# alibaba-mmai-research/CLIP-FSAR

Hardware: AMD Instinct MI355X
Metric: episodes/sec (5-way 1-shot, 8 frames, ViT-B/16) (higher is better)
Workload: dtype bf16; 1 GPU; BASELINE config[1]: 5-way 1-shot, 1 query/class, 8x224^2 frames, ViT-B/16, random-init CLIP weights, synthetic structured frames; frames_per_episode=80, precision=bf16, parallelism=episodes sharded over 1 rank(s); one all-gather of accuracies, launcher=single process

## Files before the change

clip-fsar_amd/csrc/gemm_vit.hip:

```cpp
#include <type_traits>
#include <utility>

#include "common.h"
#include "gemm_vit.h"

#include "gemm_vit_epi.h"

namespace {

template <typename TI, typename TO, int ACT, int MODE, int OPATH, int STORE, bool SHORTK = false, int MIW = 4>
__global__ __launch_bounds__(512, 2) void vit_gemm_kernel(VitGemmArgs p) {
    static_assert(!SHORTK || OPATH == 1, "K = 128 runs on the LDS-DMA path");
    static_assert(MIW == 4 || (MIW == 3 && !SHORTK), "tile height 256 or 192");
    constexpr int TMv = 64 * MIW;
    constexpr int WR = 32 * MIW;
    constexpr int NM = 2 * MIW;
    constexpr int NL = MIW + 2;
    constexpr bool WIDE = MODE == 6;
    constexpr bool HAS_RES = MODE == 1 || WIDE;
    constexpr bool LNFOLD = MODE == 2 || MODE == 4;
    constexpr bool HB = MODE == 4;
    extern __shared__ __attribute__((aligned(16))) char smem[];
    const int tid = threadIdx.x, lane = tid & 63;
    const int wave = __builtin_amdgcn_readfirstlane(tid >> 6);
    const int wm = wave >> 2, wn = wave & 3;
    const int lr = lane & 31, hi = lane >> 5;

// ... 219 lines not shown
    };
    u32x4 GX[4], GW[4];
    uint4 xfA[4], wfA[2], xfB[4], wfB[2];
    auto gloadX = [&](const unsigned (&ox)[4], int kt, auto J) __attribute__((always_inline)) {
        GX[decltype(J)::value] = *reinterpret_cast<const u32x4*>(p.A + (size_t)(kt >= p.nka ? kt - p.nka : kt) * akstride + ox[decltype(J)::value]);
    };
    auto gloadW = [&](const unsigned (&ow)[4], int kt, auto J) __attribute__((always_inline)) {
        GW[decltype(J)::value] = *reinterpret_cast<const u32x4*>(p.W + (size_t)kt * ROWB + ow[decltype(J)::value]);
    };
    auto swriteX = [&](int stage, auto J) __attribute__((always_inline)) {
        *reinterpret_cast<u32x4*>(smem + stage * STAGE + wr_off + decltype(J)::value * 8192) = GX[decltype(J)::value];
    };
    auto swriteW = [&](int stage, auto J) __attribute__((always_inline)) {
        *reinterpret_cast<u32x4*>(smem + stage * STAGE + TM * ROWB + wr_off + decltype(J)::value * 8192) = GW[decltype(J)::value];
    };
    auto dmaX = [&](const unsigned (&ox)[4], int kt, int stage, auto J) __attribute__((always_inline)) {
        const char* src = p.A + (size_t)(kt >= p.nka ? kt - p.nka : kt) * akstride + ox[decltype(J)::value];
        const unsigned dst = ldsw + (unsigned)stage * (unsigned)STAGE + (unsigned)decltype(J)::value * 8192u;
#ifdef CFSAR_DEV
        if (p.dbg & 4096) { glds16_asm_pol<1>(src, dst); return; }
        if (p.dbg & 16384) { glds16_asm_pol<2>(src, dst); return; }
#endif
        glds16_asm(src, dst);
    };
    auto dmaW = [&](const unsigned (&ow)[4], int kt, int stage, auto J) __attribute__((always_inline)) {
        const char* src = p.W + (size_t)kt * ROWB + ow[decltype(J)::value];
        const unsigned dst = ldsw + (unsigned)stage * (unsigned)STAGE + (unsigned)(TM * ROWB) + (unsigned)decltype(J)::value * 8192u;
#ifdef CFSAR_DEV
        if (p.dbg & 8192) { glds16_asm_pol<1>(src, dst); return; }
#endif
        glds16_asm(src, dst);
    };
    using T_ = std::true_type;
    using F_ = std::false_type;
    auto load_one = [&](int stage, int ss, auto J, uint4 (&xf)[4], uint4 (&wf)[2]) __attribute__((always_inline)) {
        constexpr int j = decltype(J)::value;
        const char* base = smem + stage * STAGE;
        const int x2 = ss << 5;
        constexpr int isx[6] = {1, 0, 1, 1, MIW == 4 ? 1 : 0, 0};
        constexpr int idx[6] = {0, 0, 1, 2, MIW == 4 ? 3 : 1, 1};
        if constexpr (isx[j] != 0) xf[idx[j]] = *reinterpret_cast<const uint4*>(base + (rdX[idx[j]] ^ x2));
        else wf[idx[j]] = *reinterpret_cast<const uint4*>(base + (rdW[idx[j]] ^ x2));
    };
    auto mfma_one = [&](auto J, uint4 (&xf)[4], uint4 (&wf)[2], auto ZERO) __attribute__((always_inline)) {
        constexpr int j = decltype(J)::value;
        constexpr int ni = j / MIW, mi = j % MIW;
        const f32x16 zero = {0.f, 0.f, 0.f, 0.f, 0.f, 0.f, 0.f, 0.f, 0.f, 0.f, 0.f, 0.f, 0.f, 0.f, 0.f, 0.f};
        const f32x16 c = decltype(ZERO)::value ? zero : acc[mi][ni];
        if constexpr (std::is_same<TI, _Float16>::value)
            acc[mi][ni] = __builtin_amdgcn_mfma_f32_32x32x16_f16(__builtin_bit_cast(f16x8, wf[ni]), __builtin_bit_cast(f16x8, xf[mi]), c, 0, 0, 0);
        else
            acc[mi][ni] = __builtin_amdgcn_mfma_f32_32x32x16_bf16(__builtin_bit_cast(bf16x8, wf[ni]), __builtin_bit_cast(bf16x8, xf[mi]), c, 0, 0, 0);
    };
    auto step = [&](int cur, int nxt, const unsigned (&ox)[4], const unsigned (&ow)[4], int ksrc, auto LOAD, auto WRITE, auto SYNC, auto FRAGS, auto ZERO, auto TAIL, int kstat = -1) __attribute__((always_inline)) {
        constexpr bool load = decltype(LOAD)::value, write = decltype(WRITE)::value, sync = decltype(SYNC)::value,
                       frags = decltype(FRAGS)::value, tail = decltype(TAIL)::value;
        static_for<NM>([&](auto J) {
            constexpr int j = decltype(J)::value;
            mfma_one(J, xfA, wfA, ZERO);
            if constexpr (j < NL) load_one(cur, 1, J, xfB, wfB);
            if constexpr (j >= NM - MIW) {
                if constexpr (OPATH == 0) { if constexpr (write) swriteX(nxt, std::integral_constant<int, j - (NM - MIW)>{}); }
                else if constexpr (OPATH == 1) { if constexpr (load) dmaX(ox, ksrc, nxt, std::integral_constant<int, j - (NM - MIW)>{}); }
            }
            __builtin_amdgcn_sched_barrier(0);
        });
        static_for<NM>([&](auto J) {
            constexpr int j = decltype(J)::value;
            mfma_one(J, xfB, wfB, F_{});
            if constexpr (j < NL) load_one(cur, 2, J, xfA, wfA);
            if constexpr (OPATH == 0) {
                if constexpr (j >= NM - MIW && load) gloadX(ox, ksrc, std::integral_constant<int, j - (NM - MIW)>{});
            } else if constexpr (OPATH == 1) {
                if constexpr (j >= NM - 4 && load) dmaW(ow, ksrc, nxt, std::integral_constant<int, j - (NM - 4)>{});
            }
            __builtin_amdgcn_sched_barrier(0);
        });
        static_for<NM>([&](auto J) {
            constexpr int j = decltype(J)::value;
            mfma_one(J, xfA, wfA, F_{});
            if constexpr (j < NL) load_one(cur, 3, J, xfB, wfB);
            if constexpr (j >= NM - 4 && OPATH == 0 && write) swriteW(nxt, std::integral_constant<int, j - (NM - 4)>{});
            __builtin_amdgcn_sched_barrier(0);
        });
        static_for<NM>([&](auto J) {
            constexpr int j = decltype(J)::value;
            mfma_one(J, xfB, wfB, F_{});
            if constexpr (j < 2) {
                if constexpr (OPATH == 0 && load) {
                    gloadW(ow, ksrc, std::integral_constant<int, 2 * j>{});
                    gloadW(ow, ksrc, std::integral_constant<int, 2 * j + 1>{});
                }
            } else if constexpr (frags) {
                load_one(nxt, 0, std::integral_constant<int, j - 2>{}, xfA, wfA);
                if constexpr (j == NM - 1 && NL > NM - 2) load_one(nxt, 0, std::integral_constant<int, NL - 1>{}, xfA, wfA);
            }
            if constexpr (tail && j == 2) tail_loads(m0, n0);
            if constexpr (kFuseStats && j == 2) stats_at(kstat);
            if constexpr (OPATH == 2 && load && j >= 2 && MIW == 4) {
                if constexpr (j < 6) dmaX(ox, ksrc, cur, std::integral_constant<int, j - 2>{});
                else {
                    dmaW(ow, ksrc, cur, std::integral_constant<int, 2 * (j - 6)>{});
                    dmaW(ow, ksrc, cur, std::integral_constant<int, 2 * (j - 6) + 1>{});
                }
            }
            if constexpr (OPATH == 2 && load && j >= 2 && MIW == 3) {
                if constexpr (j == 2) { dmaX(ox, ksrc, cur, std::integral_constant<int, 0>{}); dmaX(ox, ksrc, cur, std::integral_constant<int, 1>{}); }
                if constexpr (j == 3) { dmaX(ox, ksrc, cur, std::integral_constant<int, 2>{}); dmaW(ow, ksrc, cur, std::integral_constant<int, 0>{}); }
                if constexpr (j == 4) { dmaW(ow, ksrc, cur, std::integral_constant<int, 1>{}); dmaW(ow, ksrc, cur, std::integral_constant<int, 2>{}); }
                if constexpr (j == 5) { dmaW(ow, ksrc, cur, std::integral_constant<int, 3>{}); }
            }
            __builtin_amdgcn_sched_barrier(0);
            if constexpr (j == 1 && sync) {
                if constexpr (OPATH >= 1) asm volatile("s_waitcnt vmcnt(0)" ::: "memory");
#ifndef CFSAR_HIDDEN_TAIL_LOADS
                if constexpr (!frags && OPATH >= 1) tail_pin();
#endif
                __syncthreads();
                __builtin_amdgcn_sched_barrier(0);
            }
        });
    };
    origin(b, m0, n0);
    unsigned offX[4], offW[4];
    offsets(m0, n0, offX, offW);
    if constexpr (OPATH == 0) {
        static_for<MIW>([&](auto J) { gloadX(offX, 0, J); });
        static_for<4>([&](auto J) { gloadW(offW, 0, J); });
        static_for<MIW>([&](auto J) { swriteX(0, J); });
        static_for<4>([&](auto J) { swriteW(0, J); });
        static_for<MIW>([&](auto J) { gloadX(offX, 1, J); });
        static_for<4>([&](auto J) { gloadW(offW, 1, J); });
    } else {
        static_for<MIW>([&](auto J) { dmaX(offX, 0, 0, J); });
        static_for<4>([&](auto J) { dmaW(offW, 0, 0, J); });
        if constexpr (OPATH == 2) {
            static_for<MIW>([&](auto J) { dmaX(offX, 1, 1, J); });
            static_for<4>([&](auto J) { dmaW(offW, 1, 1, J); });
            asm volatile("s_waitcnt vmcnt(%0)" : : "n"(MIW + 4) : "memory");
        } else {
            asm volatile("s_waitcnt vmcnt(0)" ::: "memory");
        }
    }
    __syncthreads();
#ifdef CFSAR_DEV
    if (p.dbg & 32768) {
        if (wave >= 4) __builtin_amdgcn_s_setprio(1);
    }
    if (p.dbg & 65536) {
        if (wave < 4) __builtin_amdgcn_s_setprio(1);
    }
#endif
    int sb = 0;
// ... 2 lines not shown
    int trace_i = 0;
    if (p.dbg & 128) {
        const int n = ((blockIdx.x >> 3) & 31) * p.stagger_unit;
        for (int i = 0; i < n; ++i) __builtin_amdgcn_s_sleep(1);
        __syncthreads();
    }
#define CFSAR_TRACE(slot) do { if (p.trace && tid == 0 && trace_i < 64) p.trace[((size_t)blockIdx.x * 64 + trace_i) * 4 + (slot)] = (long long)__builtin_amdgcn_s_memrealtime(); } while (0)
#else
#define CFSAR_TRACE(slot) do { } while (0)
#endif
    for (;;) {
        const int bn = b + grid;
        const bool has_next = bn < nt;
        int m0n = m0, n0n = n0;
        if (has_next) origin(bn, m0n, n0n);
        static_for<NL>([&](auto J) { load_one(sb, 0, J, xfA, wfA); });
        CFSAR_TRACE(0);
        int kt = 0;
        u32x4 rv0[4] = {};
        auto residual_prefetch = [&]() __attribute__((always_inline)) {
            if constexpr (HAS_RES && !WIDE && OPATH >= 1) {
                const int mb_ = m0 + wm * WR, nb_ = n0 + wn * 64;
                const int ncl_ = nb_ + 64 <= p.N ? nb_ : p.N - 64;
                const int rr_ = lane >> 3, Q_ = lane & 7;
#pragma unroll
                for (int it = 0; it < 4; ++it) {
                    int row = mb_ + rr_ + it * 8;
                    row = row < p.M ? row : p.M - 1;
                    rv0[it] = *reinterpret_cast<const u32x4*>(reinterpret_cast<const char*>(p.res) + ((size_t)row * p.ldr + ncl_ + 8 * Q_) * 2);
                }
            }
        };
        if constexpr (OPATH == 0) {
            step(sb & 1, (sb + 1) & 1, offX, offW, 2, T_{}, T_{}, T_{}, T_{}, T_{}, F_{});
            for (kt = 1; kt < nk - 2; ++kt) step((sb + kt) & 1, (sb + kt + 1) & 1, offX, offW, kt + 2, T_{}, T_{}, T_{}, T_{}, F_{}, F_{});
            offsets(m0n, n0n, offX, offW);
            step((sb + kt) & 1, (sb + kt + 1) & 1, offX, offW, 0, T_{}, T_{}, T_{}, T_{}, F_{}, T_{});
            ++kt;
            step((sb + kt) & 1, (sb + kt + 1) & 1, offX, offW, 1, T_{}, T_{}, T_{}, F_{}, F_{}, F_{});
            asm volatile("s_waitcnt vmcnt(%0)" : : "n"(MIW + 4) : "memory");
        } else if constexpr (OPATH == 1 && SHORTK) {
            step(sb & 1, (sb + 1) & 1, offX, offW, 1, T_{}, F_{}, T_{}, T_{}, T_{}, T_{});
            kt = 1;
            offsets(m0n, n0n, offX, offW);
            residual_prefetch();
            step((sb + kt) & 1, (sb + kt + 1) & 1, offX, offW, 0, T_{}, F_{}, T_{}, F_{}, F_{}, F_{});
        } else if constexpr (OPATH == 1) {
            step(sb & 1, (sb + 1) & 1, offX, offW, 1, T_{}, F_{}, T_{}, T_{}, T_{}, F_{});
            for (kt = 1; kt < nk - 2; ++kt) step((sb + kt) & 1, (sb + kt + 1) & 1, offX, offW, kt + 1, T_{}, F_{}, T_{}, T_{}, F_{}, F_{});
            step((sb + kt) & 1, (sb + kt + 1) & 1, offX, offW, kt + 1, T_{}, F_{}, T_{}, T_{}, F_{}, T_{});
            ++kt;
            offsets(m0n, n0n, offX, offW);
            residual_prefetch();
            step((sb + kt) & 1, (sb + kt + 1) & 1, offX, offW, 0, T_{}, F_{}, T_{}, F_{}, F_{}, F_{});
        } else {
            step(sb & 1, (sb + 1) & 1, offX, offW, 2, T_{}, F_{}, T_{}, T_{}, T_{}, F_{}, 0);
            for (kt = 1; kt < nk - 2; ++kt) step((sb + kt) & 1, (sb + kt + 1) & 1, offX, offW, kt + 2, T_{}, F_{}, T_{}, T_{}, F_{}, F_{}, kt);
            offsets(m0n, n0n, offX, offW);
            step((sb + kt) & 1, (sb + kt + 1) & 1, offX, offW, 0, T_{}, F_{}, T_{}, T_{}, F_{}, T_{});
            ++kt;
            residual_prefetch();
// ... 42 lines not shown

int vit_pick_miw(int M, int tiles_n, int mode, int opath, int K, int dbg) {
    if (K == 128 || !vit_has_192(mode, opath)) return 4;
    const long long G = persistent_grid();
    const long long t256 = (long long)((M + 255) / 256) * tiles_n, t192 = (long long)((M + 191) / 192) * tiles_n;
    const long long r256 = ((t256 + G - 1) / G) * 256, r192 = ((t192 + G - 1) / G) * 192;
    int miw = r192 * 10 <= r256 * 9 ? 3 : 4;
#ifdef CFSAR_DEV
    if (dbg & (1 << 17)) miw = 3;
    if (dbg & (1 << 18)) miw = 4;
#endif
    (void)dbg;
    return miw;
}

template <typename TI, typename TO, int ACT, int MODE, int OPATH, int STORE, bool SHORTK, int MIW = 4>
int launch_inst2(const VitGemmArgs& a, hipStream_t s) {
    auto* fn = &vit_gemm_kernel<TI, TO, ACT, MODE, OPATH, STORE, SHORTK, MIW>;
    if (int rc = cfsar_ensure_lds(reinterpret_cast<const void*>(fn), LDS_BYTES, "cfsar_gemm(vit)")) return rc;
    const int grid = a.ntiles < persistent_grid() ? ((a.ntiles + 7) & ~7) : persistent_grid();
    hipLaunchKernelGGL(fn, dim3(grid), dim3(512), LDS_BYTES, s, a);
    return cfsar_check_launch("cfsar_gemm(vit)");
}

template <typename TI, typename TO, int ACT, int MODE, int OPATH, int STORE>
int launch_inst(const VitGemmArgs& a, hipStream_t s) {
    if (a.K == 128) return launch_inst2<TI, TO, ACT, MODE, 1, STORE, true>(a, s);
    if constexpr (vit_has_192(MODE, OPATH)) {
        if (a.miw == 3) return launch_inst2<TI, TO, ACT, MODE, OPATH, STORE, false, 3>(a, s);
    }
    return launch_inst2<TI, TO, ACT, MODE, OPATH, STORE, false>(a, s);
}

template <int OPATH, int STORE>
int launch_path(const VitGemmArgs& a, int mode, bool f16io, hipStream_t s) {
    if constexpr (STORE == 0) {
        if (mode == 5) return launch_inst<__bf16, __bf16, CFSAR_ACT_NONE, 1, OPATH, STORE>(a, s);
        if (mode == 6) return launch_inst<_Float16, _Float16, CFSAR_ACT_NONE, 6, OPATH, STORE>(a, s);
        if (mode == 1) {
            if (f16io) return launch_inst<_Float16, _Float16, CFSAR_ACT_NONE, 1, OPATH, STORE>(a, s);
            return launch_inst<__bf16, _Float16, CFSAR_ACT_NONE, 1, OPATH, STORE>(a, s);
        }
    } else {
        if (mode == 2) {
            if (f16io) {
                if (a.hb_tokens > 0) return -2;
                if (a.act == CFSAR_ACT_QUICKGELU) return launch_inst<_Float16, _Float16, CFSAR_ACT_QUICKGELU, 2, OPATH, STORE>(a, s);
                return launch_inst<_Float16, _Float16, CFSAR_ACT_NONE, 2, OPATH, STORE>(a, s);
            }
            if (a.act == CFSAR_ACT_QUICKGELU) return launch_inst<_Float16, __bf16, CFSAR_ACT_QUICKGELU, 2, OPATH, STORE>(a, s);
            if (a.hb_tokens > 0) return launch_inst<_Float16, __bf16, CFSAR_ACT_NONE, 4, OPATH, STORE>(a, s);
            return launch_inst<_Float16, __bf16, CFSAR_ACT_NONE, 2, OPATH, STORE>(a, s);
        }
        if (mode == 0) {
            if (a.act == CFSAR_ACT_QUICKGELU) return launch_inst<__bf16, __bf16, CFSAR_ACT_QUICKGELU, 0, OPATH, STORE>(a, s);
            if (a.relu) return launch_inst<__bf16, __bf16, kActRelu, 0, OPATH, STORE>(a, s);
            return launch_inst<__bf16, __bf16, CFSAR_ACT_NONE, 0, OPATH, STORE>(a, s);
        }
    }
    return cfsar_fail("cfsar_gemm (vit): internal: no instance of mode %d with store policy %d", mode, STORE);
}

}

#ifdef CFSAR_DEV
static int g_stagger_unit = 0;
static long long* g_trace = nullptr;
#endif
int cfsar_gemm_vit_try(const VitGemmCall& c, hipStream_t s) {
    const bool lnfold = c.rowstats != nullptr || c.part != nullptr;
    const bool f16io = lnfold ? c.out_dtype == CFSAR_F16 : c.in_dtype == CFSAR_F16;
    const bool f16res = !lnfold && c.out_dtype == CFSAR_F16 && c.res && c.res_dtype == CFSAR_F16 && c.act == CFSAR_ACT_NONE;
// ... 49 lines not shown
    a.ntiles = ((c.M + 64 * a.miw - 1) / (64 * a.miw)) * a.tiles_n;
    a.group = c.pol.group;
    a.colfast = c.pol.colfast;
    a.hb_tokens = c.hb_tokens; a.hb_heads = c.hb_heads; a.ha_tokens = c.ha_tokens;
    if (a.hb_tokens > 0 && !(lnfold && c.act == CFSAR_ACT_NONE && a.hb_tokens >= 128 && a.hb_heads > 0 && c.N == 3 * 64 * a.hb_heads &&
                             c.M % a.hb_tokens == 0))
        return cfsar_fail("cfsar_gemm_lnfold: head-blocked output needs act NONE, N = 192 heads, tokens >= 128, M a multiple of tokens");
    if (a.ha_tokens > 0 && !(f16res && a.ha_tokens >= 8 && c.M % a.ha_tokens == 0))
        return cfsar_fail("cfsar_gemm_residual_stats: head-blocked A needs M a multiple of tokens");
#ifdef CFSAR_DEV
    a.dbg = c.dbg;
    a.stagger_unit = g_stagger_unit;
    a.trace = g_trace;
#endif
    const int mode = lnfold ? 2 : (f16res ? (c.wide ? 6 : 1) : (bf16res ? 5 : 0));
    switch (c.pol.opath * 4 + c.pol.store) {
        case 0: return launch_path<0, 0>(a, mode, f16io, s);
        case 2: return launch_path<0, 2>(a, mode, f16io, s);
        case 8: return launch_path<2, 0>(a, mode, f16io, s);
        case 10: return launch_path<2, 2>(a, mode, f16io, s);
        default: return cfsar_fail("cfsar_gemm (vit): operand path %d / store policy %d is not built", c.pol.opath, c.pol.store);
    }
}

#ifdef CFSAR_DEV
static int g_force_opath = -1, g_force_dbg = 0;
#endif
VitPolicy cfsar_vit_policy(VitLaunchKind kind, int K) {
    const bool longk = K > 1024;
    const bool gemm = kind == kVitGemmPlain || kind == kVitGemmResidual;
    VitPolicy pol;
    pol.opath = longk ? 0 : 2;
    pol.store = (kind == kVitLnfold || kind == kVitGemmPlain) ? 2 : 0;
    pol.group = gemm ? 8 : (longk ? 16 : 6);
    pol.colfast = !gemm && longk;
// ... 12 lines not shown

namespace {
__global__ __launch_bounds__(256) void frame_means_from_colsums_kernel(const int* __restrict__ cs, __bf16* __restrict__ out, int wr,
                                                                       int tokens, int N) {
    const int f = blockIdx.y, n = blockIdx.x * 256 + threadIdx.x;
    if (n >= N) return;
    const int r0 = f * tokens, r1 = r0 + tokens - 1;
    long long s = 0;
    for (int b = r0 / wr; b <= r1 / wr; ++b) {
        const int j = f - (b * wr) / tokens;
        if (j == 0 || j == 1) s += cs[((size_t)b * 2 + j) * N + n];
    }
    out[(size_t)f * N + n] = (__bf16)((float)s * (1.0f / 4096.0f) / (float)tokens);
}
}

static int gemm_lnfold_impl(const void* x, const void* Wg, void* out, const float* cvec, const float* dvec,
                            const float* rowstats, int M, int N, int K, int lda, int ldw, int ldo, int act, int out_dtype, int hb_tokens,
                            int hb_heads, cfsar_stream_t stream, const float* partial = nullptr, int slots = 0, float eps = 0.f, int wsplit = 0,
                            const float* corr = nullptr, int corr_tokens = 0, void* colmean_out = nullptr, void* colsum_ws = nullptr) {
    CFSAR_REQUIRE(out_dtype == CFSAR_BF16 || out_dtype == CFSAR_F16, "cfsar_gemm_lnfold: out_dtype must be bf16 or fp16, got %d", out_dtype);
    CFSAR_REQUIRE(x && Wg && out && cvec && dvec && (rowstats || partial), "cfsar_gemm_lnfold: null pointer");
    CFSAR_REQUIRE(M > 0 && N > 0 && K >= 128 && K % 64 == 0 && N % 64 == 0, "cfsar_gemm_lnfold: bad shape M=%d N=%d K=%d (K %% 64, N %% 64, K >= 128)", M, N, K);
    CFSAR_REQUIRE(lda >= K && ldw >= (wsplit ? 2 * K : K) && ldo >= N && lda % 8 == 0 && ldw % 8 == 0 && ldo % 8 == 0, "cfsar_gemm_lnfold: bad leading dimension");
    CFSAR_REQUIRE(act == CFSAR_ACT_NONE || act == CFSAR_ACT_QUICKGELU, "cfsar_gemm_lnfold: bad act %d", act);
    const int ka_ = K;
    if (wsplit) K = 2 * K;
    VitGemmCall c;
    c.ka = ka_;
    c.corr_raw = corr_tokens < 0;
    if (corr_tokens < 0) corr_tokens = -corr_tokens;
    c.corr = corr; c.corr_tokens = corr_tokens;
    int miw_used = 4;
    c.colsum = colmean_out ? colsum_ws : nullptr; c.out_miw = &miw_used;
    c.A = x; c.W = Wg; c.out = out; c.bias = dvec; c.res = nullptr; c.rowstats = partial ? nullptr : rowstats; c.cvec = cvec; c.stats_out = nullptr;
    c.part = partial; c.part_slots = slots; c.part_eps = eps;
    c.M = M; c.N = N; c.K = K; c.lda = lda; c.ldw = ldw; c.ldo = ldo; c.ldr = 0;
    c.out_dtype = out_dtype; c.in_dtype = CFSAR_F16; c.res_dtype = CFSAR_F32; c.act = act; c.relu = 0;
    c.pol = cfsar_vit_policy(kVitLnfold, ka_); c.dbg = 0;
    c.hb_tokens = hb_tokens; c.hb_heads = hb_heads; c.ha_tokens = 0;
#ifdef CFSAR_DEV
    c.dbg = g_force_dbg;
#endif
    const int rc = cfsar_gemm_vit_try(c, static_cast<hipStream_t>(stream));
    if (rc == 0 && colmean_out) {
        const int frames = (M + corr_tokens - 1) / corr_tokens;
        hipLaunchKernelGGL(frame_means_from_colsums_kernel, dim3((unsigned)((N + 255) / 256), (unsigned)frames), dim3(256), 0,
                           static_cast<hipStream_t>(stream), static_cast<const int*>(colsum_ws), static_cast<__bf16*>(colmean_out),
                           32 * miw_used, corr_tokens, N);
        return cfsar_check_launch("cfsar_gemm_lnfold_hp(frame means)");
    }
    return rc == -2 ? cfsar_fail("cfsar_gemm_lnfold: operands too large for 32-bit offsets") : rc;
}

// ... 10 lines not shown
                  "cfsar_gemm_lnfold_heads: needs tokens >= 128, N = 192 heads, M a multiple of tokens (M=%d N=%d tokens=%d heads=%d)", M, N,
                  tokens, heads);
    return gemm_lnfold_impl(x, Wg, out, cvec, dvec, rowstats, M, N, K, lda, ldw, N, CFSAR_ACT_NONE, CFSAR_BF16, tokens, heads, stream);
}

static int lnfold_partials_impl(const void* x, const void* Wg, void* out, const float* cvec, const float* dvec,
                                const float* partial, int slots, float eps, float* rowstats_ws, int M, int N, int K, int lda,
                                int ldw, int ldo, int act, int out_dtype, int tokens, int heads, int wsplit, cfsar_stream_t stream,
                                const float* corr = nullptr, int corr_tokens = 0, void* colmean_out = nullptr, void* colsum_ws = nullptr) {
    CFSAR_REQUIRE(partial != nullptr && rowstats_ws != nullptr, "cfsar_gemm_lnfold_partials: null partials / workspace");
    CFSAR_REQUIRE(slots > 0 && slots * 64 == K, "cfsar_gemm_lnfold_partials: K=%d is not 64 x slots=%d", K, slots);
    int dbg = 0;
#ifdef CFSAR_DEV
    dbg = g_force_dbg;
#endif
    const int opath = cfsar_vit_policy(kVitLnfold, K).opath;
    const bool fused = !wsplit && opath == 2 && (slots == 12 || slots == 16) && vit_pick_miw(M, (N + TN - 1) / TN, 2, opath, K, dbg) == 3;
    if (!fused) {
        if (int rc = cfsar_ln_stats_finalize(partial, rowstats_ws, M, slots, K, eps, stream)) return rc;
        if (tokens > 0) return cfsar_gemm_lnfold_heads(x, Wg, out, cvec, dvec, rowstats_ws, M, N, K, lda, ldw, tokens, heads, stream);
        return gemm_lnfold_impl(x, Wg, out, cvec, dvec, rowstats_ws, M, N, K, lda, ldw, ldo, act, out_dtype, 0, 0, stream, nullptr, 0, 0.f, wsplit, corr, corr_tokens,
                                colmean_out, colsum_ws);
    }
    if (tokens > 0) {
        CFSAR_REQUIRE(tokens >= 128 && heads > 0 && N == 192 * heads && M % tokens == 0 && act == CFSAR_ACT_NONE && out_dtype == CFSAR_BF16,
                      "cfsar_gemm_lnfold_partials: head-blocked output needs tokens >= 128, N = 192 heads, M a multiple of tokens, act NONE, bf16");
        return gemm_lnfold_impl(x, Wg, out, cvec, dvec, nullptr, M, N, K, lda, ldw, N, act, out_dtype, tokens, heads, stream, partial, slots, eps);
    }
    return gemm_lnfold_impl(x, Wg, out, cvec, dvec, nullptr, M, N, K, lda, ldw, ldo, act, out_dtype, 0, 0, stream, partial, slots, eps, wsplit, corr, corr_tokens,
                            colmean_out, colsum_ws);
}
// ... 23 lines not shown

static int gemm_residual_stats_impl(const void* A, const void* W, void* x, const float* bias, float* stats_partial, int M,
                                    int N, int K, int lda, int ldw, int ldx, int in_dtype, int ha_tokens, cfsar_stream_t stream) {
    CFSAR_REQUIRE(in_dtype == CFSAR_BF16 || in_dtype == CFSAR_F16, "cfsar_gemm_residual_stats: in_dtype must be bf16 or fp16, got %d", in_dtype);
    CFSAR_REQUIRE(A && W && x && bias, "cfsar_gemm_residual_stats: null pointer");
    CFSAR_REQUIRE(M > 0 && N > 0 && K >= 128 && K % 64 == 0 && N % 64 == 0, "cfsar_gemm_residual_stats: bad shape M=%d N=%d K=%d", M, N, K);
    CFSAR_REQUIRE(lda >= K && ldw >= K && ldx >= N && lda % 8 == 0 && ldw % 8 == 0 && ldx % 8 == 0, "cfsar_gemm_residual_stats: bad leading dimension");
    VitGemmCall c;
    c.A = A; c.W = W; c.out = x; c.bias = bias; c.res = x; c.rowstats = nullptr; c.cvec = nullptr; c.stats_out = stats_partial;
    c.part = nullptr; c.part_slots = 0; c.part_eps = 0.f;
    c.M = M; c.N = N; c.K = K; c.lda = lda; c.ldw = ldw; c.ldo = ldx; c.ldr = ldx;
    c.out_dtype = CFSAR_F16; c.in_dtype = in_dtype; c.res_dtype = CFSAR_F16; c.act = CFSAR_ACT_NONE; c.relu = 0;
    c.pol = cfsar_vit_policy(kVitResidual, K); c.dbg = 0;
    c.hb_tokens = 0; c.hb_heads = 0; c.ha_tokens = ha_tokens;
#ifdef CFSAR_DEV
    c.dbg = g_force_dbg & ((1 << 17) | (1 << 18));
#endif
    const int rc = cfsar_gemm_vit_try(c, static_cast<hipStream_t>(stream));
    return rc == -2 ? cfsar_fail("cfsar_gemm_residual_stats: operands too large for 32-bit offsets") : rc;
}

extern "C" int cfsar_gemm_residual_stats(const void* A, const void* W, void* x, const float* bias, float* stats_partial, int M,
                                         int N, int K, int lda, int ldw, int ldx, int in_dtype, cfsar_stream_t stream) {
    return gemm_residual_stats_impl(A, W, x, bias, stats_partial, M, N, K, lda, ldw, ldx, in_dtype, 0, stream);
}

extern "C" int cfsar_gemm_residual_wide(const void* A, const void* W, void* x_hi, void* x_lo, const float* bias, float* stats_partial, int M,
                                        int N, int K, int wsplit, int lda, int ldw, int ldx, const float* corr, int corr_tokens,
                                        cfsar_stream_t stream) {
    CFSAR_REQUIRE(corr == nullptr || corr_tokens >= 128, "cfsar_gemm_residual_wide: the per-frame correction needs >= 128 tokens per frame");
    CFSAR_REQUIRE(A && W && x_hi && bias, "cfsar_gemm_residual_wide: null pointer");
    CFSAR_REQUIRE(M > 0 && N > 0 && K >= 128 && K % 64 == 0 && N % 64 == 0, "cfsar_gemm_residual_wide: bad shape M=%d N=%d K=%d", M, N, K);
    CFSAR_REQUIRE(wsplit >= 0 && wsplit <= 2, "cfsar_gemm_residual_wide: wsplit must be 0, 1 or 2, got %d", wsplit);
    CFSAR_REQUIRE(wsplit != 2 || corr == nullptr, "cfsar_gemm_residual_wide: wsplit = 2 carries the weights' second word itself (no per-frame correction)");
    const int Kt = wsplit == 2 ? 3 * K : (wsplit ? 2 * K : K);
    const int Ka = wsplit == 2 ? 2 * K : K;
    CFSAR_REQUIRE(lda >= Ka && ldw >= Kt && ldx >= N && lda % 8 == 0 && ldw % 8 == 0 && ldx % 8 == 0, "cfsar_gemm_residual_wide: bad leading dimension");
    VitGemmCall c;
    c.A = A; c.W = W; c.out = x_hi; c.bias = bias; c.res = x_hi; c.rowstats = nullptr; c.cvec = nullptr; c.stats_out = stats_partial;
    c.part = nullptr; c.part_slots = 0; c.part_eps = 0.f;
    c.M = M; c.N = N; c.K = Kt; c.lda = lda; c.ldw = ldw; c.ldo = ldx; c.ldr = ldx;
    c.out_dtype = CFSAR_F16; c.in_dtype = CFSAR_F16; c.res_dtype = CFSAR_F16; c.act = CFSAR_ACT_NONE; c.relu = 0;
    c.pol = cfsar_vit_policy(kVitWide, K); c.dbg = 0;
    c.hb_tokens = 0; c.hb_heads = 0; c.ha_tokens = 0;
    c.ka = Ka; c.wide = 1; c.res_lo = x_lo; c.corr = corr; c.corr_tokens = corr_tokens;
#ifdef CFSAR_DEV
    c.dbg = g_force_dbg & ((1 << 17) | (1 << 18));
#endif
    const int rc = cfsar_gemm_vit_try(c, static_cast<hipStream_t>(stream));
    return rc == -2 ? cfsar_fail("cfsar_gemm_residual_wide: operands too large for 32-bit offsets") : rc;
}

extern "C" int cfsar_gemm_residual_stats_heads(const void* A, const void* W, void* x, const float* bias, float* stats_partial, int M,
                                               int N, int K, int ldw, int ldx, int tokens, cfsar_stream_t stream) {
    CFSAR_REQUIRE(tokens >= 8 && M % tokens == 0, "cfsar_gemm_residual_stats_heads: M=%d is not a multiple of tokens=%d", M, tokens);
    return gemm_residual_stats_impl(A, W, x, bias, stats_partial, M, N, K, K, ldw, ldx, CFSAR_BF16, tokens, stream);
}
```

Before: 359.3 episodes/s.

## Add triple-buffered deep-operand ring to the early-DMA ViT GEMM pipeline

```diff
diff --git a/clip-fsar_amd/csrc/gemm_vit.hip b/clip-fsar_amd/csrc/gemm_vit.hip
--- a/clip-fsar_amd/csrc/gemm_vit.hip
+++ b/clip-fsar_amd/csrc/gemm_vit.hip
@@ -5,12 +5,15 @@
 #include "gemm_vit.h"
 
 #include "gemm_vit_epi.h"
+#include "gemm_vit_ring.h"
 
 namespace {
 
-template <typename TI, typename TO, int ACT, int MODE, int OPATH, int STORE, bool SHORTK = false, int MIW = 4>
+template <typename TI, typename TO, int ACT, int MODE, int OPATH, int STORE, bool SHORTK = false, int MIW = 4, int DEEP = 0>
 __global__ __launch_bounds__(512, 2) void vit_gemm_kernel(VitGemmArgs p) {
     static_assert(!SHORTK || OPATH == 1, "K = 128 runs on the LDS-DMA path");
+    static_assert(DEEP == 0 || (OPATH == 2 && MIW == 4 && !SHORTK), "the third operand buffer: early-DMA path, 256-row tiles");
+    static_assert(8 * EPI_SLAB == TM * ROWB, "the slab area holds one 256-row operand tile");
     static_assert(MIW == 4 || (MIW == 3 && !SHORTK), "tile height 256 or 192");
     constexpr int TMv = 64 * MIW;
     constexpr int WR = 32 * MIW;
@@ -260,18 +263,18 @@
     auto swriteW = [&](int stage, auto J) __attribute__((always_inline)) {
         *reinterpret_cast<u32x4*>(smem + stage * STAGE + TM * ROWB + wr_off + decltype(J)::value * 8192) = GW[decltype(J)::value];
     };
-    auto dmaX = [&](const unsigned (&ox)[4], int kt, int stage, auto J) __attribute__((always_inline)) {
+    auto dmaX = [&](const unsigned (&ox)[4], int kt, unsigned adst, auto J) __attribute__((always_inline)) {
         const char* src = p.A + (size_t)(kt >= p.nka ? kt - p.nka : kt) * akstride + ox[decltype(J)::value];
-        const unsigned dst = ldsw + (unsigned)stage * (unsigned)STAGE + (unsigned)decltype(J)::value * 8192u;
+        const unsigned dst = ldsw + adst + (unsigned)decltype(J)::value * 8192u;
 #ifdef CFSAR_DEV
         if (p.dbg & 4096) { glds16_asm_pol<1>(src, dst); return; }
         if (p.dbg & 16384) { glds16_asm_pol<2>(src, dst); return; }
 #endif
         glds16_asm(src, dst);
     };
-    auto dmaW = [&](const unsigned (&ow)[4], int kt, int stage, auto J) __attribute__((always_inline)) {
+    auto dmaW = [&](const unsigned (&ow)[4], int kt, unsigned wdst, auto J) __attribute__((always_inline)) {
         const char* src = p.W + (size_t)kt * ROWB + ow[decltype(J)::value];
-        const unsigned dst = ldsw + (unsigned)stage * (unsigned)STAGE + (unsigned)(TM * ROWB) + (unsigned)decltype(J)::value * 8192u;
+        const unsigned dst = ldsw + wdst + (unsigned)(TM * ROWB) + (unsigned)decltype(J)::value * 8192u;
 #ifdef CFSAR_DEV
         if (p.dbg & 8192) { glds16_asm_pol<1>(src, dst); return; }
 #endif
@@ -279,14 +282,15 @@
     };
     using T_ = std::true_type;
     using F_ = std::false_type;
-    auto load_one = [&](int stage, int ss, auto J, uint4 (&xf)[4], uint4 (&wf)[2]) __attribute__((always_inline)) {
+    auto load_one = [&](int aoff, int woff, int ss, auto J, uint4 (&xf)[4], uint4 (&wf)[2]) __attribute__((always_inline)) {
         constexpr int j = decltype(J)::value;
-        const char* base = smem + stage * STAGE;
+        const char* abase = smem + aoff;
+        const char* wbase = smem + woff;
         const int x2 = ss << 5;
         constexpr int isx[6] = {1, 0, 1, 1, MIW == 4 ? 1 : 0, 0};
         constexpr int idx[6] = {0, 0, 1, 2, MIW == 4 ? 3 : 1, 1};
-        if constexpr (isx[j] != 0) xf[idx[j]] = *reinterpret_cast<const uint4*>(base + (rdX[idx[j]] ^ x2));
-        else wf[idx[j]] = *reinterpret_cast<const uint4*>(base + (rdW[idx[j]] ^ x2));
+        if constexpr (isx[j] != 0) xf[idx[j]] = *reinterpret_cast<const uint4*>(abase + (rdX[idx[j]] ^ x2));
+        else wf[idx[j]] = *reinterpret_cast<const uint4*>(wbase + (rdW[idx[j]] ^ x2));
     };
     auto mfma_one = [&](auto J, uint4 (&xf)[4], uint4 (&wf)[2], auto ZERO) __attribute__((always_inline)) {
         constexpr int j = decltype(J)::value;
@@ -304,28 +308,28 @@
         static_for<NM>([&](auto J) {
             constexpr int j = decltype(J)::value;
             mfma_one(J, xfA, wfA, ZERO);
-            if constexpr (j < NL) load_one(cur, 1, J, xfB, wfB);
+            if constexpr (j < NL) load_one(cur * STAGE, cur * STAGE, 1, J, xfB, wfB);
             if constexpr (j >= NM - MIW) {
                 if constexpr (OPATH == 0) { if constexpr (write) swriteX(nxt, std::integral_constant<int, j - (NM - MIW)>{}); }
-                else if constexpr (OPATH == 1) { if constexpr (load) dmaX(ox, ksrc, nxt, std::integral_constant<int, j - (NM - MIW)>{}); }
+                else if constexpr (OPATH == 1) { if constexpr (load) dmaX(ox, ksrc, (unsigned)nxt * (unsigned)STAGE, std::integral_constant<int, j - (NM - MIW)>{}); }
             }
             __builtin_amdgcn_sched_barrier(0);
         });
         static_for<NM>([&](auto J) {
             constexpr int j = decltype(J)::value;
             mfma_one(J, xfB, wfB, F_{});
-            if constexpr (j < NL) load_one(cur, 2, J, xfA, wfA);
+            if constexpr (j < NL) load_one(cur * STAGE, cur * STAGE, 2, J, xfA, wfA);
             if constexpr (OPATH == 0) {
                 if constexpr (j >= NM - MIW && load) gloadX(ox, ksrc, std::integral_constant<int, j - (NM - MIW)>{});
             } else if constexpr (OPATH == 1) {
-                if constexpr (j >= NM - 4 && load) dmaW(ow, ksrc, nxt, std::integral_constant<int, j - (NM - 4)>{});
+                if constexpr (j >= NM - 4 && load) dmaW(ow, ksrc, (unsigned)nxt * (unsigned)STAGE, std::integral_constant<int, j - (NM - 4)>{});
             }
             __builtin_amdgcn_sched_barrier(0);
         });
         static_for<NM>([&](auto J) {
             constexpr int j = decltype(J)::value;
             mfma_one(J, xfA, wfA, F_{});
-            if constexpr (j < NL) load_one(cur, 3, J, xfB, wfB);
+            if constexpr (j < NL) load_one(cur * STAGE, cur * STAGE, 3, J, xfB, wfB);
             if constexpr (j >= NM - 4 && OPATH == 0 && write) swriteW(nxt, std::integral_constant<int, j - (NM - 4)>{});
             __builtin_amdgcn_sched_barrier(0);
         });
@@ -338,23 +342,23 @@
                     gloadW(ow, ksrc, std::integral_constant<int, 2 * j + 1>{});
                 }
             } else if constexpr (frags) {
-                load_one(nxt, 0, std::integral_constant<int, j - 2>{}, xfA, wfA);
-                if constexpr (j == NM - 1 && NL > NM - 2) load_one(nxt, 0, std::integral_constant<int, NL - 1>{}, xfA, wfA);
+                load_one(nxt * STAGE, nxt * STAGE, 0, std::integral_constant<int, j - 2>{}, xfA, wfA);
+                if constexpr (j == NM - 1 && NL > NM - 2) load_one(nxt * STAGE, nxt * STAGE, 0, std::integral_constant<int, NL - 1>{}, xfA, wfA);
             }
             if constexpr (tail && j == 2) tail_loads(m0, n0);
             if constexpr (kFuseStats && j == 2) stats_at(kstat);
             if constexpr (OPATH == 2 && load && j >= 2 && MIW == 4) {
-                if constexpr (j < 6) dmaX(ox, ksrc, cur, std::integral_constant<int, j - 2>{});
+                if constexpr (j < 6) dmaX(ox, ksrc, (unsigned)cur * (unsigned)STAGE, std::integral_constant<int, j - 2>{});
                 else {
-                    dmaW(ow, ksrc, cur, std::integral_constant<int, 2 * (j - 6)>{});
-                    dmaW(ow, ksrc, cur, std::integral_constant<int, 2 * (j - 6) + 1>{});
+                    dmaW(ow, ksrc, (unsigned)cur * (unsigned)STAGE, std::integral_constant<int, 2 * (j - 6)>{});
+                    dmaW(ow, ksrc, (unsigned)cur * (unsigned)STAGE, std::integral_constant<int, 2 * (j - 6) + 1>{});
                 }
             }
             if constexpr (OPATH == 2 && load && j >= 2 && MIW == 3) {
-                if constexpr (j == 2) { dmaX(ox, ksrc, cur, std::integral_constant<int, 0>{}); dmaX(ox, ksrc, cur, std::integral_constant<int, 1>{}); }
-                if constexpr (j == 3) { dmaX(ox, ksrc, cur, std::integral_constant<int, 2>{}); dmaW(ow, ksrc, cur, std::integral_constant<int, 0>{}); }
-                if constexpr (j == 4) { dmaW(ow, ksrc, cur, std::integral_constant<int, 1>{}); dmaW(ow, ksrc, cur, std::integral_constant<int, 2>{}); }
-                if constexpr (j == 5) { dmaW(ow, ksrc, cur, std::integral_constant<int, 3>{}); }
+                if constexpr (j == 2) { dmaX(ox, ksrc, (unsigned)cur * (unsigned)STAGE, std::integral_constant<int, 0>{}); dmaX(ox, ksrc, (unsigned)cur * (unsigned)STAGE, std::integral_constant<int, 1>{}); }
+                if constexpr (j == 3) { dmaX(ox, ksrc, (unsigned)cur * (unsigned)STAGE, std::integral_constant<int, 2>{}); dmaW(ow, ksrc, (unsigned)cur * (unsigned)STAGE, std::integral_constant<int, 0>{}); }
+                if constexpr (j == 4) { dmaW(ow, ksrc, (unsigned)cur * (unsigned)STAGE, std::integral_constant<int, 1>{}); dmaW(ow, ksrc, (unsigned)cur * (unsigned)STAGE, std::integral_constant<int, 2>{}); }
+                if constexpr (j == 5) { dmaW(ow, ksrc, (unsigned)cur * (unsigned)STAGE, std::integral_constant<int, 3>{}); }
             }
             __builtin_amdgcn_sched_barrier(0);
             if constexpr (j == 1 && sync) {
@@ -363,6 +367,79 @@
                 if constexpr (!frags && OPATH >= 1) tail_pin();
 #endif
                 __syncthreads();
+                __builtin_amdgcn_sched_barrier(0);
+            }
+        });
+    };
+
+    auto d_off = [&](int buf) __attribute__((always_inline)) -> int {
+        int off = buf == vit_ring::kSlab ? (DEEP == 2 ? EPI_OFF - TM * ROWB : EPI_OFF) : buf * STAGE;
+        asm volatile("" : "+s"(off));
+        return off;
+    };
+    auto step_deep = [&](int k, int sb_, const unsigned (&ox)[4], const unsigned (&ow)[4], auto KIND, auto KREP) __attribute__((always_inline)) {
+        constexpr int kind = decltype(KIND)::value;
+        using ZERO = std::integral_constant<bool, kind == 0>;
+        constexpr vit_ring::Step rd = vit_ring::step(decltype(KREP)::value, vit_ring::kRepTiles);
+        static_assert(kind == (rd.d_tile[1] != vit_ring::kNone ? 0 : rd.leave_d_tiles ? (rd.d_tile[0] != vit_ring::kNone ? 1 : 2) : (rd.d_dst[0] == 0 ? 3 : 4)), "step kind and ring step disagree");
+        const vit_ring::Step r = vit_ring::step(k, nk);
+        const int dcur = d_off(rd.d_read), scur = ((r.s_read + sb_) & 1) * STAGE;
+        const int dnxt = d_off(rd.d_next), snxt = ((r.s_next + sb_) & 1) * STAGE;
+        const int acur = DEEP == 1 ? dcur : scur, wcur = DEEP == 1 ? scur : dcur;
+        const int anxt = DEEP == 1 ? dnxt : snxt, wnxt = DEEP == 1 ? snxt : dnxt;
+        const int st = r.s_tile >= nk ? r.s_tile - nk : r.s_tile;
+        const unsigned sdst = (unsigned)(((r.s_dst + sb_) & 1) * STAGE);
+        auto issueS = [&](auto J) __attribute__((always_inline)) {
+            if constexpr (DEEP == 1) dmaW(ow, st, sdst, J); else dmaX(ox, st, sdst, J);
+        };
+        auto issueD = [&](int which, auto J) __attribute__((always_inline)) {
+            const int dt = r.d_tile[which] >= nk ? r.d_tile[which] - nk : r.d_tile[which];
+            const unsigned ddst = (unsigned)d_off(rd.d_dst[which]);
+            if constexpr (DEEP == 1) dmaX(ox, dt, ddst, J); else dmaW(ow, dt, ddst, J);
+        };
+        static_for<NM>([&](auto J) {
+            mfma_one(J, xfA, wfA, ZERO{});
+            if constexpr (decltype(J)::value < NL) load_one(acur, wcur, 1, J, xfB, wfB);
+            __builtin_amdgcn_sched_barrier(0);
+        });
+        static_for<NM>([&](auto J) {
+            mfma_one(J, xfB, wfB, F_{});
+            if constexpr (decltype(J)::value < NL) load_one(acur, wcur, 2, J, xfA, wfA);
+            __builtin_amdgcn_sched_barrier(0);
+        });
+        static_for<NM>([&](auto J) {
+            mfma_one(J, xfA, wfA, F_{});
+            if constexpr (decltype(J)::value < NL) load_one(acur, wcur, 3, J, xfB, wfB);
+            __builtin_amdgcn_sched_barrier(0);
+        });
+        static_for<NM>([&](auto J) {
+            constexpr int j = decltype(J)::value;
+            mfma_one(J, xfB, wfB, F_{});
+            if constexpr (j >= 2 && kind != 4) load_one(anxt, wnxt, 0, std::integral_constant<int, j - 2>{}, xfA, wfA);
+            if constexpr (kind == 3 && j == 2) tail_loads(m0, n0);
+            if constexpr (kind == 0 && j >= 2) {
+                constexpr int q = 2 * ((j - 2) & 1);
+                if constexpr (j < 4) { issueS(std::integral_constant<int, q>{}); issueS(std::integral_constant<int, q + 1>{}); }
+                else { issueD((j - 4) >> 1, std::integral_constant<int, q>{}); issueD((j - 4) >> 1, std::integral_constant<int, q + 1>{}); }
+            }
+            if constexpr (kind != 0 && j >= 2) {
+                if constexpr (j < 6) issueS(std::integral_constant<int, j - 2>{});
+                else if constexpr (kind != 2) { issueD(0, std::integral_constant<int, 2 * (j - 6)>{}); issueD(0, std::integral_constant<int, 2 * (j - 6) + 1>{}); }
+            }
+            __builtin_amdgcn_sched_barrier(0);
+            if constexpr (j == 1) {
+                if constexpr (kind == 1 || kind == 2) {
+                    asm volatile("s_waitcnt vmcnt(%0)" : : "n"(MIW) : "memory");
+                    asm volatile("s_waitcnt lgkmcnt(0)" ::: "memory");
+                    __builtin_amdgcn_s_barrier();
+                    asm volatile("" ::: "memory");
+                } else {
+                    asm volatile("s_waitcnt vmcnt(0)" ::: "memory");
+#ifndef CFSAR_HIDDEN_TAIL_LOADS
+                    if constexpr (kind == 4) tail_pin();
+#endif
+                    __syncthreads();
+                }
                 __builtin_amdgcn_sched_barrier(0);
             }
         });
@@ -378,11 +455,11 @@
         static_for<MIW>([&](auto J) { gloadX(offX, 1, J); });
         static_for<4>([&](auto J) { gloadW(offW, 1, J); });
     } else {
-        static_for<MIW>([&](auto J) { dmaX(offX, 0, 0, J); });
-        static_for<4>([&](auto J) { dmaW(offW, 0, 0, J); });
+        static_for<MIW>([&](auto J) { dmaX(offX, 0, 0u, J); });
+        static_for<4>([&](auto J) { dmaW(offW, 0, 0u, J); });
         if constexpr (OPATH == 2) {
-            static_for<MIW>([&](auto J) { dmaX(offX, 1, 1, J); });
-            static_for<4>([&](auto J) { dmaW(offW, 1, 1, J); });
+            static_for<MIW>([&](auto J) { dmaX(offX, 1, (unsigned)STAGE, J); });
+            static_for<4>([&](auto J) { dmaW(offW, 1, (unsigned)STAGE, J); });
             asm volatile("s_waitcnt vmcnt(%0)" : : "n"(MIW + 4) : "memory");
         } else {
             asm volatile("s_waitcnt vmcnt(0)" ::: "memory");
@@ -415,7 +492,9 @@
         const bool has_next = bn < nt;
         int m0n = m0, n0n = n0;
         if (has_next) origin(bn, m0n, n0n);
-        static_for<NL>([&](auto J) { load_one(sb, 0, J, xfA, wfA); });
+        static_for<NL>([&](auto J) {
+            load_one(DEEP == 1 ? 0 : sb * STAGE, DEEP == 2 ? 0 : sb * STAGE, 0, J, xfA, wfA);
+        });
         CFSAR_TRACE(0);
         int kt = 0;
         u32x4 rv0[4] = {};
@@ -446,6 +525,25 @@
             offsets(m0n, n0n, offX, offW);
             residual_prefetch();
             step((sb + kt) & 1, (sb + kt + 1) & 1, offX, offW, 0, T_{}, F_{}, T_{}, F_{}, F_{}, F_{});
+        } else if constexpr (DEEP != 0) {
+            using I0 = std::integral_constant<int, 0>; using I1 = std::integral_constant<int, 1>; using I2 = std::integral_constant<int, 2>;
+            using I3 = std::integral_constant<int, 3>; using I4 = std::integral_constant<int, 4>; using I5 = std::integral_constant<int, 5>;
+            constexpr int RT = vit_ring::kRepTiles;
+            step_deep(0, sb, offX, offW, I0{}, I0{});
+            step_deep(1, sb, offX, offW, I1{}, I4{});
+            step_deep(2, sb, offX, offW, I1{}, I5{});
+            for (kt = 3; kt < nk - 3; kt += 3) {
+                step_deep(kt, sb, offX, offW, I1{}, I3{});
+                step_deep(kt + 1, sb, offX, offW, I1{}, I4{});
+                step_deep(kt + 2, sb, offX, offW, I1{}, I5{});
+            }
+            step_deep(kt, sb, offX, offW, I2{}, std::integral_constant<int, RT - 3>{});
+            ++kt;
+            offsets(m0n, n0n, offX, offW);
+            step_deep(kt, sb, offX, offW, I3{}, std::integral_constant<int, RT - 2>{});
+            ++kt;
+            residual_prefetch();
+            step_deep(kt, sb, offX, offW, I4{}, std::integral_constant<int, RT - 1>{});
         } else if constexpr (OPATH == 1) {
             step(sb & 1, (sb + 1) & 1, offX, offW, 1, T_{}, F_{}, T_{}, T_{}, T_{}, F_{});
             for (kt = 1; kt < nk - 2; ++kt) step((sb + kt) & 1, (sb + kt + 1) & 1, offX, offW, kt + 1, T_{}, F_{}, T_{}, T_{}, F_{}, F_{});
@@ -518,9 +616,19 @@
     return miw;
 }
 
-template <typename TI, typename TO, int ACT, int MODE, int OPATH, int STORE, bool SHORTK, int MIW = 4>
+int vit_pick_deep(int opath, int miw, int K, bool fused_stats, int dbg) {
+    int deep = (opath == 2 && miw == 4 && K != 128 && !fused_stats && vit_ring::eligible(K / 64)) ? 1 : 0;
+#ifdef CFSAR_DEV
+    if (deep && (dbg & (1 << 23))) deep = 0;
+    if (deep && (dbg & (1 << 24))) deep = 2;
+#endif
+    (void)dbg;
+    return deep;
+}
+
+template <typename TI, typename TO, int ACT, int MODE, int OPATH, int STORE, bool SHORTK, int MIW = 4, int DEEP = 0>
 int launch_inst2(const VitGemmArgs& a, hipStream_t s) {
-    auto* fn = &vit_gemm_kernel<TI, TO, ACT, MODE, OPATH, STORE, SHORTK, MIW>;
+    auto* fn = &vit_gemm_kernel<TI, TO, ACT, MODE, OPATH, STORE, SHORTK, MIW, DEEP>;
     if (int rc = cfsar_ensure_lds(reinterpret_cast<const void*>(fn), LDS_BYTES, "cfsar_gemm(vit)")) return rc;
     const int grid = a.ntiles < persistent_grid() ? ((a.ntiles + 7) & ~7) : persistent_grid();
     hipLaunchKernelGGL(fn, dim3(grid), dim3(512), LDS_BYTES, s, a);
@@ -528,38 +636,49 @@
 }
 
 template <typename TI, typename TO, int ACT, int MODE, int OPATH, int STORE>
-int launch_inst(const VitGemmArgs& a, hipStream_t s) {
+int launch_inst(const VitGemmArgs& a, int deep, hipStream_t s) {
     if (a.K == 128) return launch_inst2<TI, TO, ACT, MODE, 1, STORE, true>(a, s);
     if constexpr (vit_has_192(MODE, OPATH)) {
         if (a.miw == 3) return launch_inst2<TI, TO, ACT, MODE, OPATH, STORE, false, 3>(a, s);
     }
+#ifdef CFSAR_DEV
+    constexpr bool kRing = OPATH == 2;
+#else
+    constexpr bool kRing = OPATH == 2 && !(MODE == 0 && ACT == CFSAR_ACT_QUICKGELU);
+#endif
+    if constexpr (kRing) {
+        if (deep == 1) return launch_inst2<TI, TO, ACT, MODE, OPATH, STORE, false, 4, 1>(a, s);
+#ifdef CFSAR_DEV
+        if (deep == 2) return launch_inst2<TI, TO, ACT, MODE, OPATH, STORE, false, 4, 2>(a, s);
+#endif
+    }
     return launch_inst2<TI, TO, ACT, MODE, OPATH, STORE, false>(a, s);
 }
 
 template <int OPATH, int STORE>
-int launch_path(const VitGemmArgs& a, int mode, bool f16io, hipStream_t s) {
+int launch_path(const VitGemmArgs& a, int deep, int mode, bool f16io, hipStream_t s) {
     if constexpr (STORE == 0) {
-        if (mode == 5) return launch_inst<__bf16, __bf16, CFSAR_ACT_NONE, 1, OPATH, STORE>(a, s);
-        if (mode == 6) return launch_inst<_Float16, _Float16, CFSAR_ACT_NONE, 6, OPATH, STORE>(a, s);
+        if (mode == 5) return launch_inst<__bf16, __bf16, CFSAR_ACT_NONE, 1, OPATH, STORE>(a, deep, s);
+        if (mode == 6) return launch_inst<_Float16, _Float16, CFSAR_ACT_NONE, 6, OPATH, STORE>(a, deep, s);
         if (mode == 1) {
-            if (f16io) return launch_inst<_Float16, _Float16, CFSAR_ACT_NONE, 1, OPATH, STORE>(a, s);
-            return launch_inst<__bf16, _Float16, CFSAR_ACT_NONE, 1, OPATH, STORE>(a, s);
+            if (f16io) return launch_inst<_Float16, _Float16, CFSAR_ACT_NONE, 1, OPATH, STORE>(a, deep, s);
+            return launch_inst<__bf16, _Float16, CFSAR_ACT_NONE, 1, OPATH, STORE>(a, deep, s);
         }
     } else {
         if (mode == 2) {
             if (f16io) {
                 if (a.hb_tokens > 0) return -2;
-                if (a.act == CFSAR_ACT_QUICKGELU) return launch_inst<_Float16, _Float16, CFSAR_ACT_QUICKGELU, 2, OPATH, STORE>(a, s);
-                return launch_inst<_Float16, _Float16, CFSAR_ACT_NONE, 2, OPATH, STORE>(a, s);
-            }
-            if (a.act == CFSAR_ACT_QUICKGELU) return launch_inst<_Float16, __bf16, CFSAR_ACT_QUICKGELU, 2, OPATH, STORE>(a, s);
-            if (a.hb_tokens > 0) return launch_inst<_Float16, __bf16, CFSAR_ACT_NONE, 4, OPATH, STORE>(a, s);
-            return launch_inst<_Float16, __bf16, CFSAR_ACT_NONE, 2, OPATH, STORE>(a, s);
+                if (a.act == CFSAR_ACT_QUICKGELU) return launch_inst<_Float16, _Float16, CFSAR_ACT_QUICKGELU, 2, OPATH, STORE>(a, deep, s);
+                return launch_inst<_Float16, _Float16, CFSAR_ACT_NONE, 2, OPATH, STORE>(a, deep, s);
+            }
+            if (a.act == CFSAR_ACT_QUICKGELU) return launch_inst<_Float16, __bf16, CFSAR_ACT_QUICKGELU, 2, OPATH, STORE>(a, deep, s);
+            if (a.hb_tokens > 0) return launch_inst<_Float16, __bf16, CFSAR_ACT_NONE, 4, OPATH, STORE>(a, deep, s);
+            return launch_inst<_Float16, __bf16, CFSAR_ACT_NONE, 2, OPATH, STORE>(a, deep, s);
         }
         if (mode == 0) {
-            if (a.act == CFSAR_ACT_QUICKGELU) return launch_inst<__bf16, __bf16, CFSAR_ACT_QUICKGELU, 0, OPATH, STORE>(a, s);
-            if (a.relu) return launch_inst<__bf16, __bf16, kActRelu, 0, OPATH, STORE>(a, s);
-            return launch_inst<__bf16, __bf16, CFSAR_ACT_NONE, 0, OPATH, STORE>(a, s);
+            if (a.act == CFSAR_ACT_QUICKGELU) return launch_inst<__bf16, __bf16, CFSAR_ACT_QUICKGELU, 0, OPATH, STORE>(a, deep, s);
+            if (a.relu) return launch_inst<__bf16, __bf16, kActRelu, 0, OPATH, STORE>(a, deep, s);
+            return launch_inst<__bf16, __bf16, CFSAR_ACT_NONE, 0, OPATH, STORE>(a, deep, s);
         }
     }
     return cfsar_fail("cfsar_gemm (vit): internal: no instance of mode %d with store policy %d", mode, STORE);
@@ -639,11 +758,12 @@
     a.trace = g_trace;
 #endif
     const int mode = lnfold ? 2 : (f16res ? (c.wide ? 6 : 1) : (bf16res ? 5 : 0));
+    const int deep = vit_pick_deep(c.pol.opath, a.miw, c.K, c.part != nullptr, c.dbg);
     switch (c.pol.opath * 4 + c.pol.store) {
-        case 0: return launch_path<0, 0>(a, mode, f16io, s);
-        case 2: return launch_path<0, 2>(a, mode, f16io, s);
-        case 8: return launch_path<2, 0>(a, mode, f16io, s);
-        case 10: return launch_path<2, 2>(a, mode, f16io, s);
+        case 0: return launch_path<0, 0>(a, deep, mode, f16io, s);
+        case 2: return launch_path<0, 2>(a, deep, mode, f16io, s);
+        case 8: return launch_path<2, 0>(a, deep, mode, f16io, s);
+        case 10: return launch_path<2, 2>(a, deep, mode, f16io, s);
         default: return cfsar_fail("cfsar_gemm (vit): operand path %d / store policy %d is not built", c.pol.opath, c.pol.store);
     }
 }
@@ -686,6 +806,8 @@
     out[(size_t)f * N + n] = (__bf16)((float)s * (1.0f / 4096.0f) / (float)tokens);
 }
 }
+
+static VitPolicy lnfold_policy(int ka) { return cfsar_vit_policy(kVitLnfold, ka); }
 
 static int gemm_lnfold_impl(const void* x, const void* Wg, void* out, const float* cvec, const float* dvec,
                             const float* rowstats, int M, int N, int K, int lda, int ldw, int ldo, int act, int out_dtype, int hb_tokens,
@@ -709,7 +831,7 @@
     c.part = partial; c.part_slots = slots; c.part_eps = eps;
     c.M = M; c.N = N; c.K = K; c.lda = lda; c.ldw = ldw; c.ldo = ldo; c.ldr = 0;
     c.out_dtype = out_dtype; c.in_dtype = CFSAR_F16; c.res_dtype = CFSAR_F32; c.act = act; c.relu = 0;
-    c.pol = cfsar_vit_policy(kVitLnfold, ka_); c.dbg = 0;
+    c.pol = lnfold_policy(ka_); c.dbg = 0;
     c.hb_tokens = hb_tokens; c.hb_heads = hb_heads; c.ha_tokens = 0;
 #ifdef CFSAR_DEV
     c.dbg = g_force_dbg;
@@ -750,7 +872,7 @@
 #ifdef CFSAR_DEV
     dbg = g_force_dbg;
 #endif
-    const int opath = cfsar_vit_policy(kVitLnfold, K).opath;
+    const int opath = lnfold_policy(K).opath;
     const bool fused = !wsplit && opath == 2 && (slots == 12 || slots == 16) && vit_pick_miw(M, (N + TN - 1) / TN, 2, opath, K, dbg) == 3;
     if (!fused) {
         if (int rc = cfsar_ln_stats_finalize(partial, rowstats_ws, M, slots, K, eps, stream)) return rc;
@@ -804,7 +926,7 @@
     c.pol = cfsar_vit_policy(kVitResidual, K); c.dbg = 0;
     c.hb_tokens = 0; c.hb_heads = 0; c.ha_tokens = ha_tokens;
 #ifdef CFSAR_DEV
-    c.dbg = g_force_dbg & ((1 << 17) | (1 << 18));
+    c.dbg = g_force_dbg & ((1 << 17) | (1 << 18) | (1 << 23) | (1 << 24));
 #endif
     const int rc = cfsar_gemm_vit_try(c, static_cast<hipStream_t>(stream));
     return rc == -2 ? cfsar_fail("cfsar_gemm_residual_stats: operands too large for 32-bit offsets") : rc;
@@ -835,7 +957,7 @@
     c.hb_tokens = 0; c.hb_heads = 0; c.ha_tokens = 0;
     c.ka = Ka; c.wide = 1; c.res_lo = x_lo; c.corr = corr; c.corr_tokens = corr_tokens;
 #ifdef CFSAR_DEV
-    c.dbg = g_force_dbg & ((1 << 17) | (1 << 18));
+    c.dbg = g_force_dbg & ((1 << 17) | (1 << 18) | (1 << 23) | (1 << 24));
 #endif
     const int rc = cfsar_gemm_vit_try(c, static_cast<hipStream_t>(stream));
     return rc == -2 ? cfsar_fail("cfsar_gemm_residual_wide: operands too large for 32-bit offsets") : rc;
diff --git a/clip-fsar_amd/csrc/gemm_vit_ring.h b/clip-fsar_amd/csrc/gemm_vit_ring.h
--- /dev/null
+++ b/clip-fsar_amd/csrc/gemm_vit_ring.h
@@ -0,0 +1,110 @@
+#pragma once
+
+namespace vit_ring {
+
+constexpr int kSlab = 2;
+constexpr int kNone = -1;
+
+struct Step {
+    int d_read, s_read;
+    int d_next, s_next;
+    int s_tile, s_dst;
+    int d_tile[2], d_dst[2];
+    int leave_d_tiles;
+};
+
+constexpr Step step(int k, int nk) {
+    Step r{k % 3, k & 1, (k + 1) % 3, (k + 1) & 1, k + 2, k & 1, {kNone, kNone}, {kNone, kNone}, 0};
+    if (k == 0) {
+        r.d_tile[0] = 2; r.d_dst[0] = kSlab;
+        r.d_tile[1] = 3; r.d_dst[1] = 0;
+    } else if (k <= nk - 4) {
+        r.d_tile[0] = k + 3; r.d_dst[0] = k % 3;
+    } else if (k >= nk - 2) {
+        r.d_tile[0] = k + 2; r.d_dst[0] = k - (nk - 2);
+    }
+    r.leave_d_tiles = (k >= 1 && k <= nk - 3) ? 1 : 0;
+    return r;
+}
+
+constexpr bool eligible(int nk) { return nk >= 6 && nk % 3 == 0; }
+
+constexpr int kRepTiles = 48;
+constexpr int rep(int k, int nk) { return k == 0 ? 0 : (k <= nk - 4 ? 3 + k % 3 : kRepTiles - (nk - k)); }
+constexpr bool rep_matches(int nk) {
+    for (int k = 0; k < nk; ++k) {
+        const Step a = step(k, nk), b = step(rep(k, nk), kRepTiles);
+        if (a.d_read != b.d_read || a.d_next != b.d_next || a.leave_d_tiles != b.leave_d_tiles || (a.s_tile == kNone) != (b.s_tile == kNone)) return false;
+        for (int i = 0; i < 2; ++i)
+            if (a.d_dst[i] != b.d_dst[i] || (a.d_tile[i] == kNone) != (b.d_tile[i] == kNone)) return false;
+    }
+    return true;
+}
+
+struct Buf { int tile; bool landed, freed; };
+struct Fly { int tile, pieces, dst; bool deep; };
+constexpr int simulate(int nk, int tiles, int PD, int PS) {
+    Buf d[3] = {{0, true, false}, {1, false, false}, {kNone, false, true}};
+    Buf s[2] = {{0, true, false}, {1, false, false}};
+    Fly q[8] = {};
+    int qn = 0;
+    q[qn++] = Fly{1, PD, 1, true};
+    q[qn++] = Fly{1, PS, 1, false};
+    int sb = 0;
+    for (int t = 0; t < tiles; ++t) {
+        for (int k = 0; k < nk; ++k) {
+            const Step r = step(k, nk);
+            const int g = t * nk + k;
+            Buf& dr = d[r.d_read];
+            Buf& sr = s[(r.s_read + sb) & 1];
+            if (dr.tile != g || !dr.landed || sr.tile != g || !sr.landed) return 1;
+            const int leave = r.leave_d_tiles * PD;
+            int fly = 0;
+            for (int i = 0; i < qn; ++i) fly += q[i].pieces;
+            if (r.leave_d_tiles) {
+                if (fly <= leave || qn == 0 || !q[qn - 1].deep || q[qn - 1].pieces != leave) return 5;
+            }
+            int keep = r.leave_d_tiles ? 1 : 0;
+            for (int i = 0; i < qn - keep; ++i) {
+                Buf& b = q[i].deep ? d[q[i].dst] : s[q[i].dst];
+                if (b.tile != q[i].tile) return 3;
+                b.landed = true;
+            }
+            if (keep) q[0] = q[qn - 1];
+            qn = keep;
+            if (k == nk - 1)
+                for (int i = 0; i < qn; ++i) if (q[i].deep && q[i].dst == kSlab) return 4;
+            const Buf& dn = d[r.d_next];
+            const Buf& sn = s[(r.s_next + sb) & 1];
+            if (dn.tile != g + 1 || !dn.landed || sn.tile != g + 1 || !sn.landed) return 2;
+            dr.freed = true;
+            sr.freed = true;
+            if (r.s_tile != kNone) {
+                Buf& b = s[(r.s_dst + sb) & 1];
+                if (!b.freed) return 3;
+                b = Buf{t * nk + r.s_tile, false, false};
+                q[qn++] = Fly{b.tile, PS, (r.s_dst + sb) & 1, false};
+            }
+            for (int i = 0; i < 2; ++i) {
+                if (r.d_tile[i] == kNone) continue;
+                Buf& b = d[r.d_dst[i]];
+                if (!b.freed) return 3;
+                if (r.d_dst[i] == kSlab && k >= nk - 1) return 4;
+                b = Buf{t * nk + r.d_tile[i], false, false};
+                q[qn++] = Fly{b.tile, PD, r.d_dst[i], true};
+            }
+        }
+        sb = (sb + nk) & 1;
+    }
+    return 0;
+}
+
+static_assert(simulate(6, 4, 4, 4) == 0 && simulate(12, 4, 4, 4) == 0 && simulate(24, 3, 4, 4) == 0 && simulate(48, 3, 4, 4) == 0,
+              "deep-operand ring: a step reads, overwrites or waits for the wrong buffer");
+static_assert(simulate(9, 4, 4, 4) == 0 && simulate(15, 4, 4, 4) == 0 && simulate(36, 3, 4, 4) == 0,
+              "deep-operand ring with an odd / split-weight K tile count");
+static_assert(rep_matches(6) && rep_matches(9) && rep_matches(12) && rep_matches(15) && rep_matches(24) && rep_matches(36) && rep_matches(48),
+              "the compile-time stand-in of a step has another D side than the step");
+static_assert(eligible(6) && eligible(12) && eligible(24) && eligible(48) && !eligible(3) && !eligible(5) && !eligible(16), "eligibility by walked K tiles");
+
+}
```

Result: no change. 362.4 episodes/s (median of 6 runs) (+0.9%).
